# mll-lab-nu/TStar

Hardware: AMD Instinct MI355X
Metric: candidate frames scored/sec (whole node) + sec/video to 8 keyframes, 1h@1fps (higher is better)
Workload: dtype f32 held exactly as 3 bf16 terms per operand: every GEMM and vision-attention operand (activations, weights, Q, K, V, softmax probabilities) = three round-to-nearest bf16 terms carrying all 24 significand bits; the 6 partial products with i + j <= 2 (each exact) on v_mfma_f32_32x32x16_bf16, f32 accu

## Files before the change

### include/tstar_hip.h

```cpp
#ifndef TSTAR_HIP_H
#define TSTAR_HIP_H

#include <stddef.h>
#include <stdint.h>

#ifdef __cplusplus
extern "C" {
#endif

#define TSTAR_OK 0
#define TSTAR_ERR_ARG 1
#define TSTAR_ERR_HIP 2
#define TSTAR_ERR_STATE 3

#define TSTAR_OWL_NPATCH 576
#define TSTAR_OWL_QDIM 512
#define TSTAR_OWL_TEXT_LEN 16
#define TSTAR_OWL_MAX_QUERIES 32
#define TSTAR_OWL_MAX_SETS 64

const char* tstar_last_error(void);
int tstar_abi_version(void);
size_t tstar_owl_vision_blob_floats(void);
size_t tstar_owl_text_blob_floats(void);
// ... 109 lines not shown
int tstar_draw_boxes_np(uint8_t* d_images, int B, int H, int W, const float* d_boxes_xyxy, const float* d_scores, int np,
                        void* stream);

int tstar_gemm_f32(const float* d_A, const float* d_W, float* d_C, const float* d_bias, const float* d_residual,
                   int M, int N, int K, int act, void* stream);
int tstar_gemm_f32_cfg(const float* d_A, const float* d_W, float* d_C, const float* d_bias, const float* d_residual,
                       int M, int N, int K, int act, int tile_cfg, void* stream);
int tstar_gemm_bf16w(const float* d_A, const float* d_W, float* d_C, const float* d_bias, const float* d_residual,
                     int M, int N, int K, int act, int tile_cfg, void* stream);
int tstar_gemm_bf16w2(const float* d_A, const float* d_W, float* d_C, const float* d_bias, const float* d_residual,
                      int M, int N, int K, int act, int tile_cfg, void* stream);
int tstar_gemm_bf16w_pre(const float* d_A, const void* d_Wb, float* d_C, const float* d_bias, const float* d_residual,
                         int M, int N, int K, int act, int a_terms, int tile_cfg, void* stream);
int tstar_gemm_f32x3(const float* d_A, const float* d_W, float* d_C, const float* d_bias, const float* d_residual,
                     int M, int N, int K, int act, int tile_cfg, void* stream);
int tstar_pack_f32x3(const float* d_W, void* d_Wp, int N, int K, void* stream);
int tstar_gemm_f32x3_pre(const float* d_A, const void* d_Wp, float* d_C, const float* d_bias, const float* d_residual,
                         int M, int N, int K, int act, int tile_cfg, void* stream);
int tstar_gemm_plan(int weights_mode, int M, int N, int ldc, int patch_np, int tile_cfg, int has_packed_w2, int* plan4);
int tstar_ingest_plan(int op, int nv12, int H, int W, int n, int ow, int oh, int out_aligned4, int video_aligned4, int generic,
                      int nv12_lds, int grid_px, int* plan6);
int tstar_layernorm_f32(const float* d_x, float* d_y, const float* d_w, const float* d_b, int rows, int D, void* stream);
int tstar_attention_f32(const float* d_qkv, float* d_out, int B, int T, int heads, int mode,
                        const uint8_t* d_key_mask, void* stream);

int tstar_attention_split(const float* d_qkv, float* d_out, int B, int T, int heads, void* stream);
int tstar_attention_x3(const float* d_qkv, float* d_out, int B, int T, int heads, void* stream);

int tstar_prof_enable(int on);
int tstar_prof_read(int category, long long* launches, double* total_ms, double* total_flops);
// ... 9 lines not shown
```

### tstar_amd/_lib.py

```python
from __future__ import annotations

import ctypes as C
import os

_HERE = os.path.dirname(os.path.abspath(__file__))
LIB_PATH = os.path.join(_HERE, "libtstar_hip.so")


class TStarHipError(RuntimeError):
    pass


_vp, _i, _sz = C.c_void_p, C.c_int, C.c_size_t
_fp = C.POINTER(C.c_float)
SIGNATURES = {
    "tstar_last_error": (C.c_char_p, []),
    "tstar_abi_version": (_i, []),
    "tstar_owl_vision_blob_floats": (_sz, []),
    "tstar_owl_text_blob_floats": (_sz, []),
    "tstar_owl_create": (_i, [C.POINTER(_vp), _vp, _sz, _vp, _sz, _vp, _i, _i]),
    "tstar_owl_create_ex": (_i, [C.POINTER(_vp), _i, _i, _vp, _sz, _vp, _sz, _vp, _i, _i]),
    "tstar_owl_vision_blob_floats_ex": (_sz, [_i, _i]),
    "tstar_owl_create_in": (_i, [C.POINTER(_vp), _i, _i, _i, _vp, _sz, _vp, _sz, _vp, _i, _i]),
    "tstar_owl_vision_blob_floats_in": (_sz, [_i, _i, _i]),
# ... 40 lines not shown
    "tstar_searcher_read_state": (_i, [_vp, _vp, _vp]),
    "tstar_searcher_read": (_i, [_vp, _i, _vp, _vp]),
    "tstar_comm_available": (_i, []),
    "tstar_comm_unique_id": (_i, [_vp]),
    "tstar_comm_create": (_i, [C.POINTER(_vp), _vp, _i, _i]),
    "tstar_comm_destroy": (_i, [_vp]),
    "tstar_allgather_i32": (_i, [_vp, _vp, _vp, _i, _vp]),
    "tstar_topk_seconds": (_i, [_vp, _i, _i, _i, _i, _vp, _vp]),
    "tstar_ssim_pairwise": (_i, [_vp, _i, _vp, _i, _i, _i, _vp, _vp, _vp]),
    "tstar_gemm_f32": (_i, [_vp, _vp, _vp, _vp, _vp, _i, _i, _i, _i, _vp]),
    "tstar_gemm_f32_cfg": (_i, [_vp, _vp, _vp, _vp, _vp, _i, _i, _i, _i, _i, _vp]),
    "tstar_gemm_bf16w": (_i, [_vp, _vp, _vp, _vp, _vp, _i, _i, _i, _i, _i, _vp]),
    "tstar_gemm_bf16w2": (_i, [_vp, _vp, _vp, _vp, _vp, _i, _i, _i, _i, _i, _vp]),
    "tstar_gemm_bf16w_pre": (_i, [_vp, _vp, _vp, _vp, _vp, _i, _i, _i, _i, _i, _i, _vp]),
    "tstar_gemm_f32x3": (_i, [_vp, _vp, _vp, _vp, _vp, _i, _i, _i, _i, _i, _vp]),
    "tstar_pack_f32x3": (_i, [_vp, _vp, _i, _i, _vp]),
    "tstar_gemm_f32x3_pre": (_i, [_vp, _vp, _vp, _vp, _vp, _i, _i, _i, _i, _i, _vp]),
    "tstar_gemm_plan": (_i, [_i, _i, _i, _i, _i, _i, _i, C.POINTER(_i)]),
    "tstar_ingest_plan": (_i, [_i] * 12 + [C.POINTER(_i)]),
    "tstar_layernorm_f32": (_i, [_vp, _vp, _vp, _vp, _i, _i, _vp]),
    "tstar_draw_boxes": (_i, [_vp, _i, _i, _i, _vp, _vp, _vp]),
    "tstar_draw_boxes_np": (_i, [_vp, _i, _i, _i, _vp, _vp, _i, _vp]),
    "tstar_attention_split": (_i, [_vp, _vp, _i, _i, _i, _vp]),
    "tstar_attention_x3": (_i, [_vp, _vp, _i, _i, _i, _vp]),
    "tstar_attention_f32": (_i, [_vp, _vp, _i, _i, _i, _i, _vp, _vp]),
    "tstar_prof_enable": (_i, [_i]),
    "tstar_prof_read": (_i, [_i, _vp, _vp, _vp]),
    "tstar_prof_read_bytes": (_i, [_i, _vp]),
    "tstar_prof_read_totals": (_i, [_i, _vp, _vp]),
    "tstar_prof_mark": (_i, [_i, _vp]),
# ... 41 lines not shown
```

### tstar_amd/csrc/capi.hip

```cpp
#include "../../include/tstar_hip.h"
#include "common.h"
#include "heads.h"
#include "ingest.h"
#include "jpeg_host.h"
#include "kernels.h"
#include "owl_weights.h"
#include <math.h>
#include <map>
#include <mutex>
#include <set>
#include <string.h>
#include <unordered_map>
#include <vector>

namespace tstar {
static thread_local std::string g_err;
void set_error(const std::string& msg) { g_err = msg; }

int ensure_dyn_lds(const void* kernel, int bytes) {
    static std::mutex mu;
    static std::set<std::pair<const void*, int>> done;
    int dev = 0;
    if (hipGetDevice(&dev) != hipSuccess) { set_error("ensure_dyn_lds: hipGetDevice failed"); return 2; }
    std::lock_guard<std::mutex> lk(mu);
// ... 48 lines not shown
struct tstar_owl {
    float* d_vision = nullptr;
    float* d_text = nullptr;
    VisionW vw{};
    TextW tw{};
    bool has_text = false, has_vision = false;
    OwlGeom geom{};
    float* d_lut = nullptr;
    int max_batch = 0;
    int chunk_cap = 0;
    size_t mpad = 0;
    struct Lane {
        float *x = nullptr, *xn = nullptr, *qkv = nullptr, *att = nullptr, *hid = nullptr;
        uint8_t* tmp_u8 = nullptr; size_t tmp_u8_bytes = 0;
        int* d_image_set = nullptr; int image_set_cap = 0;
        int cap = 0;
    } lane[TSTAR_OWL_LANES];
    int Q[TSTAR_OWL_MAX_SETS] = {0};
    float *q_raw = nullptr, *qn = nullptr;
    double* qweight = nullptr;
    uint8_t* qmask = nullptr;
    int* d_setQ = nullptr;
    int *d_ids = nullptr, *d_eos = nullptr;
    uint8_t* d_kmask = nullptr;
    int seq_cap = TSTAR_OWL_MAX_QUERIES;
    std::map<std::pair<int, int>, ResampleTable> tabs;
    int weights_mode = TSTAR_WEIGHTS_F32;
    std::unordered_map<const float*, __bf16*> wb;
    std::unordered_map<const float*, void*> wp;
    std::unordered_map<const float*, void*> wq;
// ... 73 lines not shown

static GemmArgs mk_gemm(const tstar_owl* h, const float* A, const float* W, float* C, const float* bias, const float* res,
                        int M, int N, int K, int lda, int ldc, int act) {
    GemmArgs g{};
    g.A = A; g.W = W; g.Wb = h ? h->bf16_of(W) : nullptr; g.Wp = h ? h->packed_of(W) : nullptr; g.Wq = h ? h->w2_of(W) : nullptr; g.C = C; g.bias = bias; g.res = res; g.pos = nullptr;
    g.M = M; g.N = N; g.K = K; g.lda = lda; g.ldc = ldc; g.act = act; g.patch_np = 0; g.tile_cfg = TILE_AUTO; g.m_split = 0;
    g.a_terms = h && h->weights_mode == TSTAR_WEIGHTS_BF16 ? 2 : 0;
    return g;
}

static bool x3_attention_f32() {
    static const bool v = getenv("TSTAR_X3_ATTN_F32") != nullptr;
    return v;
}

static int run_encoder(tstar_owl* h, tstar_owl::Lane& L, const LayerW* layers, int nlayers, int B, int T, int D, int FF, int heads,
                       int mode, const uint8_t* key_mask, hipStream_t s) {
    const int M = B * T;
    for (int l = 0; l < nlayers; ++l) {
        const LayerW& w = layers[l];
        RC(layernorm_f32(L.x, L.xn, w.ln1_w, w.ln1_b, M, D, s));
        RC(gemm_f32(mk_gemm(h, L.xn, w.qkv_w, L.qkv, w.qkv_b, nullptr, M, 3 * D, D, D, 3 * D, ACT_NONE), s));
        if (mode == 0 && (h->weights_mode == TSTAR_WEIGHTS_BF16 || h->weights_mode == TSTAR_WEIGHTS_BF16_EXACT)) RC(attention_split(L.qkv, L.att, B, T, heads, s));
        else if (mode == 0 && h->weights_mode == TSTAR_WEIGHTS_F32X3 && !x3_attention_f32()) RC(attention_x3(L.qkv, L.att, B, T, heads, s));
        else RC(attention_f32(L.qkv, L.att, B, T, heads, mode, key_mask, s));
        RC(gemm_f32(mk_gemm(h, L.att, w.out_w, L.x, w.out_b, L.x, M, D, D, D, D, ACT_NONE), s));
        RC(layernorm_f32(L.x, L.xn, w.ln2_w, w.ln2_b, M, D, s));
        RC(gemm_f32(mk_gemm(h, L.xn, w.fc1_w, L.hid, w.fc1_b, nullptr, M, FF, D, D, FF, ACT_QGELU), s));
        RC(gemm_f32(mk_gemm(h, L.hid, w.fc2_w, L.x, w.fc2_b, L.x, M, D, FF, FF, D, ACT_NONE), s));
    }
    return TSTAR_OK;
}

static int preprocess_chunk(tstar_owl* h, tstar_owl::Lane& L, const uint8_t* d_images, int B, int H, int W, uint8_t* out_u8,
                            float* out_patches, hipStream_t s) {
    ResampleTable *th, *tv;
    const OwlGeom& G = h->geom;
    RC(get_table(h, W, G.in_w, &th, s));
    RC(get_table(h, H, G.in_h, &tv, s));
    const size_t need = (size_t)B * H * G.in_w * 3;
    if (need > L.tmp_u8_bytes) {
        TSTAR_HIP_CHECK(hipStreamSynchronize(s));
        if (L.tmp_u8) TSTAR_HIP_CHECK(hipFree(L.tmp_u8));
        L.tmp_u8 = nullptr; L.tmp_u8_bytes = 0;
        TSTAR_HIP_CHECK(hipMalloc(&L.tmp_u8, need));
        L.tmp_u8_bytes = need;
    }
    RC(resample_h_u8(d_images, L.tmp_u8, B, H, W, *th, s));
    RC(resample_v_normalize_patchify(L.tmp_u8, out_patches, out_u8, B, H, G.in_w, *tv, h->d_lut, G.patch, s));
    return TSTAR_OK;
}

static hipError_t alloc_lane(tstar_owl::Lane& L, int cap, const OwlGeom& g) {
    const size_t mp = lane_rows(cap, g);
    hipError_t e = hipSuccess;
    auto alloc = [&](float** p, size_t n) { if (e == hipSuccess) { e = hipMalloc(p, n * sizeof(float)); if (e == hipSuccess) e = hipMemset(*p, 0, n * sizeof(float)); } };
    alloc(&L.x, mp * V_D); alloc(&L.xn, mp * V_D); alloc(&L.qkv, mp * 3 * V_D); alloc(&L.att, mp * V_D); alloc(&L.hid, mp * V_FF);
    if (e == hipSuccess) L.cap = cap;
    return e;
}
static void free_lane(tstar_owl::Lane& L) {
    void* ptrs[] = {L.x, L.xn, L.qkv, L.att, L.hid, L.tmp_u8, L.d_image_set};
    for (void* p : ptrs) if (p) (void)hipFree(p);
    L = tstar_owl::Lane{};
}

extern "C" {

const char* tstar_last_error(void) { return g_err.c_str(); }
int tstar_abi_version(void) { return 3; }
size_t tstar_owl_vision_blob_floats(void) { return vision_floats(OwlGeom{}); }
size_t tstar_owl_text_blob_floats(void) { return text_floats(); }
size_t tstar_owl_vision_blob_floats_ex(int image_size, int patch_size) {
    OwlGeom g;
    if (!owl_geom(image_size, patch_size, &g)) { set_error("tstar_owl_vision_blob_floats_ex: unsupported geometry (image 768, patch 32 or 16)"); return 0; }
    return vision_floats(g);
}
// ... 356 lines not shown
        }
        TSTAR_HIP_CHECK(hipMemcpyAsync(L.d_image_set, h_image_query_set, (size_t)B * sizeof(int), hipMemcpyHostToDevice, s));
    }
    const int ncell = grid_rows * grid_cols;
    const OwlGeom& G = h->geom;
    const int NP = G.np, NTOK = G.ntok, PK = G.patch_k;
    for (int b0 = 0; b0 < B; b0 += L.cap) {
        const int Bc = (B - b0) < L.cap ? (B - b0) : L.cap;
        const int M = Bc * NTOK, MP = Bc * NP;
        RC(preprocess_chunk(h, L, d_images + (size_t)b0 * H * W * 3, Bc, H, W, nullptr, L.hid, s));
        GemmArgs pg = mk_gemm(h, L.hid, h->vw.patch_w, L.x, nullptr, nullptr, MP, V_D, PK, PK, V_D, ACT_NONE);
        pg.pos = h->vw.pos_emb; pg.patch_np = NP;
        RC(gemm_f32(pg, s));
        RC(write_cls_rows(L.x, h->vw.class_emb, h->vw.pos_emb, Bc, NTOK, V_D, s));
        RC(layernorm_f32(L.x, L.x, h->vw.pre_ln_w, h->vw.pre_ln_b, M, V_D, s));
        RC(run_encoder(h, L, h->vw.layers, V_LAYERS, Bc, NTOK, V_D, V_FF, V_HEADS, 0, nullptr, s));
        float* feats = L.xn;
        RC(merge_cls_ln(L.x, feats, h->vw.post_ln_w, h->vw.post_ln_b, h->vw.det_ln_w, h->vw.det_ln_b, Bc, NTOK, V_D, s));
        float* cls = L.att;
        float* bh1 = L.qkv;
        float* bh2 = L.hid;
        RC(gemm_f32(mk_gemm(h, feats, h->vw.cls_w, cls, h->vw.cls_b, nullptr, MP, PROJ, V_D, V_D, PROJ, ACT_NONE), s));
        RC(gemm_f32(mk_gemm(h, feats, h->vw.box0_w, bh1, h->vw.box0_b, nullptr, MP, V_D, V_D, V_D, V_D, ACT_GELU), s));
        RC(gemm_f32(mk_gemm(h, bh1, h->vw.box1_w, bh2, h->vw.box1_b, nullptr, MP, V_D, V_D, V_D, V_D, ACT_GELU), s));
        DetectRowsArgs a{};
        a.feats = feats; a.cls = cls; a.boxh = bh2; a.qn = h->qn; a.qmask = h->qmask;
        a.shift_w = h->vw.shift_w; a.shift_b = h->vw.shift_b; a.scale_w = h->vw.scale_w; a.scale_b = h->vw.scale_b;
        a.box2_w = h->vw.box2_w; a.box2_b = h->vw.box2_b; a.box_bias = h->vw.box_bias;
        a.scores = d_scores + (size_t)b0 * NP;
        a.labels = d_labels + (size_t)b0 * NP;
// ... 125 lines not shown
    void* wp = nullptr;
    TSTAR_HIP_CHECK(hipMalloc(&wp, (size_t)N * K * 6));
    int rc = pack_weights_x3(d_W, wp, N, K, s);
    if (!rc) {
        GemmArgs g = mk_gemm(nullptr, d_A, d_W, d_C, d_bias, d_residual, M, N, K, K, N, act);
        g.Wp = wp;
        g.tile_cfg = tile_cfg;
        rc = gemm_f32(g, s);
    }
    hipError_t e = hipStreamSynchronize(s);
    (void)hipFree(wp);
    if (!rc && e != hipSuccess) { set_error(std::string("tstar_gemm_f32x3: ") + hipGetErrorString(e)); rc = TSTAR_ERR_HIP; }
    return rc;
}

int tstar_pack_f32x3(const float* d_W, void* d_Wp, int N, int K, void* stream) {
    TSTAR_REQUIRE(d_W && d_Wp, "tstar_pack_f32x3: null argument");
    TSTAR_REQUIRE(N > 0 && K > 0, "tstar_pack_f32x3: empty matrix");
    return pack_weights_x3(d_W, d_Wp, N, K, (hipStream_t)stream);
}

int tstar_gemm_f32x3_pre(const float* d_A, const void* d_Wp, float* d_C, const float* d_bias, const float* d_residual, int M, int N,
                         int K, int act, int tile_cfg, void* stream) {
    TSTAR_REQUIRE(d_A && d_Wp && d_C, "tstar_gemm_f32x3_pre: null argument");
    TSTAR_REQUIRE(M > 0 && N > 0 && K > 0 && N % 128 == 0 && K % 32 == 0, "tstar_gemm_f32x3_pre: N must be a multiple of 128, K of 32 (include/tstar_hip.h)");
    GemmArgs g = mk_gemm(nullptr, d_A, reinterpret_cast<const float*>(d_Wp), d_C, d_bias, d_residual, M, N, K, K, N, act);
    g.Wp = d_Wp;
    g.tile_cfg = tile_cfg;
    return gemm_f32(g, (hipStream_t)stream);
}
// ... 54 lines not shown
```

### tstar_amd/csrc/gemm_f32.hip

```cpp
#include "common.h"
#include "kernels.h"
#include "prof.h"
#include <type_traits>
#include <utility>

namespace tstar {

constexpr int BK = 32, LDS_LD = BK + 4;

__device__ __forceinline__ void tile_mn(int tile, int mt, int nt, int gm, int& mi, int& ni) {
    if (gm <= 1) { mi = tile / nt; ni = tile - mi * nt; return; }
    const int per = gm * nt;
    const int sp = tile / per, r = tile - sp * per;
    const int left = mt - sp * gm;
    const int rows = left < gm ? left : gm;
    ni = r / rows;
    mi = sp * gm + (r - ni * rows);
}

__device__ __forceinline__ float epi_act(float v, int act) {
    if (act == ACT_QGELU) return v * __builtin_amdgcn_rcpf(1.0f + __builtin_amdgcn_exp2f(-1.702f * 1.44269504088896340736f * v));
    if (act == ACT_GELU) return 0.5f * v * (1.0f + erff(v * 0.70710678118654752440f));
    return v;
}
// ... 262 lines not shown
    __syncthreads();
    for (int kt = 0; kt < nk; kt += 2) {
        if (kt + 2 < nk) gload(S0{}, kt + 2);
        compute(0);
        if (kt + 1 < nk) lstore(S1{}, 1);
        __syncthreads();
        if (kt + 1 >= nk) break;
        if (kt + 3 < nk) gload(S1{}, kt + 3);
        compute(1);
        if (kt + 2 < nk) lstore(S0{}, 0);
        __syncthreads();
    }
    gemm_epilogue<CF, ACT, HAS_BIAS, HAS_RES, PATCH>(g, acc, m0, n0, wm, wn, l31, h);
}

template <int NA>
__device__ __forceinline__ void split4_rn(const f32x4 v, u32x2 (&out)[NA]) {
#pragma unroll
    for (int p = 0; p < 2; ++p) {
        f32x2 x; x[0] = v[2 * p]; x[1] = v[2 * p + 1];
#pragma unroll
        for (int k = 0; k < NA; ++k) {
            const bf16x2 b = __builtin_convertvector(x, bf16x2);
            const unsigned hb = __builtin_bit_cast(unsigned, b);
            out[k][p] = hb;
            if (k + 1 < NA) {
                x[0] = x[0] - __uint_as_float(hb << 16);
                x[1] = x[1] - __uint_as_float(hb & 0xFFFF0000u);
            }
        }
// ... 2 lines not shown

__device__ __forceinline__ void split2_rn3(float x0, float x1, unsigned (&o)[3]) {
#pragma unroll
    for (int k = 0; k < 3; ++k) {
        f32x2 x; x[0] = x0; x[1] = x1;
        const unsigned hb = __builtin_bit_cast(unsigned, __builtin_convertvector(x, bf16x2));
        o[k] = hb;
        if (k < 2) {
            x0 = x0 - __uint_as_float(hb << 16);
            x1 = x1 - __uint_as_float(hb & 0xFFFF0000u);
        }
    }
}

template <class CF, int ACT, bool HAS_BIAS, bool HAS_RES, bool PATCH>
__device__ __forceinline__ void gemm_tile_x3(const GemmArgs& g, const int m0, const int n0, float* smem_f) {
    constexpr int TM = CF::TM, TN = CF::TN, BM = CF::BM;
    constexpr int A_T = BM * 64, BUF = 3 * A_T;
    constexpr int NA = BM / 32;
    constexpr int PAIR = TN >= 2 ? 2 : 1, GP = TN / PAIR;
    constexpr int WD = TM * TN == 1 ? 4 : 1;
    static_assert(TN % PAIR == 0, "column tiles go in pairs");
    char* smem = reinterpret_cast<char*>(smem_f);
    const int t = threadIdx.x;
    const int lane = t & 63, wave = __builtin_amdgcn_readfirstlane(t >> 6);
    const int wm = wave >> 1, wn = wave & 1;
    const int l31 = lane & 31, h = lane >> 5;
    const int c4 = t & 7, r0 = t >> 3;
    unsigned aoff[NA];
#pragma unroll
    for (int i = 0; i < NA; ++i) {
// ... 162 lines not shown
        step(std::integral_constant<int, 1>{}, std::integral_constant<int, (s0 + 1) % WD>{}, nxt, rd0, nxt, 2 * kt + 1 + WD, 0);
    };
    if constexpr (WD <= 2) {
        for (int kt = 0; kt < nk; ++kt) tile(std::integral_constant<int, 0>{}, kt);
    } else {
        static_assert(WD == 4, "the loop below is unrolled by WD / 2 = 2 K tiles");
        int kt = 0;
        for (; kt + 1 < nk; kt += 2) {
            tile(std::integral_constant<int, 0>{}, kt);
            tile(std::integral_constant<int, 2>{}, kt + 1);
        }
        if (kt < nk) tile(std::integral_constant<int, 0>{}, kt);
    }
    __builtin_amdgcn_s_setprio(0);
    gemm_epilogue<CF, ACT, HAS_BIAS, HAS_RES, PATCH>(g, acc, m0, n0, wm, wn, l31, h);
}

__global__ __launch_bounds__(256) void pack_x3_kernel(const float* __restrict__ W, char* __restrict__ Wp, int N, int K) {
    const size_t gid = (size_t)blockIdx.x * 256 + threadIdx.x;
    const int kc = K / 8;
    if (gid >= (size_t)N * kc) return;
    const int n = (int)(gid / kc), c = (int)(gid % kc);
    const f32x4 v0 = *reinterpret_cast<const f32x4*>(W + (size_t)n * K + c * 8);
    const f32x4 v1 = *reinterpret_cast<const f32x4*>(W + (size_t)n * K + c * 8 + 4);
    u32x2 s0[3], s1[3];
    split4_rn<3>(v0, s0);
    split4_rn<3>(v1, s1);
    const int ks = c >> 1, hh = c & 1, nph = (K / 16) * 3;
#pragma unroll
    for (int ph = 0; ph < 3; ++ph) {
// ... 258 lines not shown
        __syncthreads();
        cur ^= 1;
    }

    gemm_epilogue<CF, ACT, HAS_BIAS, HAS_RES, PATCH>(g, acc, m0, n0, wm, wn, l31, h);
}

template <class CF, int WMODE, int ACT, bool HAS_BIAS, bool HAS_RES, bool PATCH>
__global__ __launch_bounds__(256, CF::MINW) void gemm_f32_kernel(GemmArgs g) {
    extern __shared__ __attribute__((aligned(16))) float smem[];
    const int nt = g.N / CF::BN;
    const int mt = (g.M + CF::BM - 1) / CF::BM;
    const int tile = xcd_remap(blockIdx.x, mt * nt);
    int mi, ni;
    tile_mn(tile, mt, nt, g.group_m, mi, ni);
    if constexpr (WMODE == 4) gemm_tile_x3<CF, ACT, HAS_BIAS, HAS_RES, PATCH>(g, mi * CF::BM, ni * CF::BN, smem);
    else if constexpr (WMODE != 0) gemm_tile_bf16w<CF, WMODE, ACT, HAS_BIAS, HAS_RES, PATCH>(g, mi * CF::BM, ni * CF::BN, smem);
    else gemm_tile<CF, ACT, HAS_BIAS, HAS_RES, PATCH>(g, mi * CF::BM, ni * CF::BN, smem);
}

template <int WMODE, int ACT, bool HAS_BIAS, bool HAS_RES, bool PATCH>
__global__ __launch_bounds__(256, 2) void gemm_f32_hybrid_kernel(GemmArgs g) {
    extern __shared__ __attribute__((aligned(16))) float smem[];
    const int nt = g.N / 128;
    const int n_big = (g.m_split / 128) * nt;
    if ((int)blockIdx.x < n_big) {
        const int tile = xcd_remap(blockIdx.x, n_big);
        int mi, ni;
        tile_mn(tile, g.m_split / 128, nt, g.group_m, mi, ni);
        if constexpr (WMODE == 4) gemm_tile_x3<Cfg128, ACT, HAS_BIAS, HAS_RES, PATCH>(g, mi * 128, ni * 128, smem);
        else if constexpr (WMODE != 0) gemm_tile_bf16w<Cfg128, WMODE, ACT, HAS_BIAS, HAS_RES, PATCH>(g, mi * 128, ni * 128, smem);
        else gemm_tile<Cfg128, ACT, HAS_BIAS, HAS_RES, PATCH>(g, mi * 128, ni * 128, smem);
    } else {
        const int n_small = gridDim.x - n_big;
        const int tile = xcd_remap(blockIdx.x - n_big, n_small);
        int mi, ni;
        tile_mn(tile, n_small / nt, nt, g.group_m, mi, ni);
        if constexpr (WMODE == 4) gemm_tile_x3<Cfg64N, ACT, HAS_BIAS, HAS_RES, PATCH>(g, g.m_split + mi * 64, ni * 128, smem);
        else if constexpr (WMODE != 0) gemm_tile_bf16w<Cfg64N, WMODE, ACT, HAS_BIAS, HAS_RES, PATCH>(g, g.m_split + mi * 64, ni * 128, smem);
        else gemm_tile<Cfg64N, ACT, HAS_BIAS, HAS_RES, PATCH>(g, g.m_split + mi * 64, ni * 128, smem);
    }
}

template <int WMODE, int ACT, bool HAS_BIAS, bool HAS_RES, bool PATCH, bool VW = false>
__global__ __launch_bounds__(256, 2) void gemm_bf16w2_wide_kernel(GemmArgs g) {
    extern __shared__ __attribute__((aligned(16))) float smem[];
    const int ntw = g.N / 256;
    const int n_big = (g.m_split / 128) * ntw;
    if ((int)blockIdx.x < n_big) {
        const int tile = xcd_remap(blockIdx.x, n_big);
        int mi, ni;
        tile_mn(tile, g.m_split / 128, ntw, g.group_m, mi, ni);
        if constexpr (WMODE == 4) gemm_tile_x3<Cfg128W, ACT, HAS_BIAS, HAS_RES, PATCH>(g, mi * 128, ni * 256, smem);
        else if constexpr (VW) gemm_tile_w2v<Cfg128W, ACT, HAS_BIAS, HAS_RES, PATCH>(g, mi * 128, ni * 256, smem);
        else gemm_tile_bf16w<Cfg128W, 3, ACT, HAS_BIAS, HAS_RES, PATCH>(g, mi * 128, ni * 256, smem);
    } else {
        const int nt = g.N / 128;
        const int n_small = gridDim.x - n_big;
        const int tile = xcd_remap(blockIdx.x - n_big, n_small);
        int mi, ni;
        tile_mn(tile, n_small / nt, nt, g.group_m, mi, ni);
        if constexpr (WMODE == 4) gemm_tile_x3<Cfg64N, ACT, HAS_BIAS, HAS_RES, PATCH>(g, g.m_split + mi * 64, ni * 128, smem);
        else gemm_tile_bf16w<Cfg64N, 3, ACT, HAS_BIAS, HAS_RES, PATCH>(g, g.m_split + mi * 64, ni * 128, smem);
    }
}

static constexpr int lds_bytes(int wmode, int bm, int bn) {
    return wmode == GEMM_W_F32X3 ? 2 * 3 * bm * 64 : wmode == GEMM_W_BF16_2T ? 2 * (2 * bm + bn) * 64 : wmode == GEMM_W_BF16_EXACT ? 2 * (3 * bm + bn) * 64 : 2 * (bm + bn) * LDS_LD * 4;
}

static double gemm_algorithmic_bytes(const GemmArgs& g) {
    const double wbytes = g.Wp ? 6.0 : g.Wb ? 2.0 : 4.0;
    return 4.0 * g.M * g.K + wbytes * g.N * g.K + 4.0 * g.M * g.N * (g.res ? 2.0 : 1.0) + (g.bias ? 4.0 * g.N : 0.0) +
           (g.pos ? 4.0 * (g.patch_np + 1) * g.N : 0.0);
}

static int pick_cfg(int M, int N, int* m_split) {
// ... 94 lines not shown
}

template <int ACT, bool HAS_BIAS, bool HAS_RES, bool PATCH>
static int launch_one(const GemmArgs& g, hipStream_t stream) {
    if (g.Wp) return launch_mode<GEMM_W_F32X3, ACT, HAS_BIAS, HAS_RES, PATCH>(g, stream);
    if (g.Wb && g.a_terms == 2) return launch_mode<GEMM_W_BF16_2T, ACT, HAS_BIAS, HAS_RES, PATCH>(g, stream);
    if (g.Wb) return launch_mode<GEMM_W_BF16_EXACT, ACT, HAS_BIAS, HAS_RES, PATCH>(g, stream);
    return launch_mode<GEMM_W_F32, ACT, HAS_BIAS, HAS_RES, PATCH>(g, stream);
}

static int default_group_m() {
    static const int gm = [] { const char* e = getenv("TSTAR_GEMM_GM"); const int v = e ? atoi(e) : 8; return v < 1 ? 1 : (v > 64 ? 64 : v); }();
    return gm;
}

int gemm_f32(const GemmArgs& g0, hipStream_t stream) {
    GemmArgs g = g0;
    if (g.group_m <= 0) g.group_m = default_group_m();
    TSTAR_REQUIRE(g.M > 0 && g.N > 0 && g.K > 0, "gemm_f32: empty problem");
    TSTAR_REQUIRE(g.K % BK == 0, "gemm_f32: K must be a multiple of 32");
    TSTAR_REQUIRE(g.lda % 4 == 0 && g.K % 4 == 0, "gemm_f32: rows must be 16-byte aligned");
    const bool bias = g.bias != nullptr, res = g.res != nullptr, patch = g.pos != nullptr;
    if (patch) {
        TSTAR_REQUIRE(!bias && !res && g.act == ACT_NONE && g.patch_np > 0, "gemm_f32: patch epilogue takes no bias/res/act");
        return launch_one<ACT_NONE, false, false, true>(g, stream);
    }
    if (g.act == ACT_QGELU) {
        TSTAR_REQUIRE(bias && !res, "gemm_f32: quick-gelu epilogue needs bias, no residual");
        return launch_one<ACT_QGELU, true, false, false>(g, stream);
    }
    if (g.act == ACT_GELU) {
        TSTAR_REQUIRE(bias && !res, "gemm_f32: gelu epilogue needs bias, no residual");
        return launch_one<ACT_GELU, true, false, false>(g, stream);
// ... 9 lines not shown
```

### tstar_amd/csrc/kernels.h

```cpp
#pragma once
#include "common.h"

namespace tstar {

enum { ACT_NONE = 0, ACT_QGELU = 1, ACT_GELU = 2 };

struct GemmArgs {
    const float* A;
    const float* W;
    const __bf16* Wb;
    const void* Wp;
    const void* Wq;
    float* C;
    const float* bias;
    const float* res;
    const float* pos;
    int M, N, K, lda, ldc;
    int act;
    int patch_np;
    int tile_cfg;
    int m_split;
    int group_m;
    int a_terms;
};
int gemm_f32(const GemmArgs& g, hipStream_t stream);

enum GemmTileCfg {
    TILE_AUTO = -1,
    TILE_128 = 0,
    TILE_64N = 1,
    TILE_64 = 2,
    TILE_HYBRID = 3,
    TILE_WIDE = 4,
    TILE_NO_WIDE = 5,
    TILE_WIDE_VW = 6,
    TILE_HYBRID_N = 16,
};

enum GemmWeightMode {
    GEMM_W_F32 = 0,
// ... 46 lines not shown
```

### tstar_amd/csrc/rowops.hip

```cpp
#include "common.h"
#include "kernels.h"

namespace tstar {

__device__ __forceinline__ float wave_sum(float v) {
#pragma unroll
    for (int o = 32; o > 0; o >>= 1) v += __shfl_xor(v, o);
    return v;
}

template <int NV>
__device__ __forceinline__ void ln_regs(f32x4 (&x)[NV], const float* __restrict__ w, const float* __restrict__ b,
                                        int lane, float invD) {
    float s = 0.f;
#pragma unroll
    for (int i = 0; i < NV; ++i) s += (x[i][0] + x[i][1]) + (x[i][2] + x[i][3]);
    const float mean = wave_sum(s) * invD;
    float v = 0.f;
#pragma unroll
    for (int i = 0; i < NV; ++i)
#pragma unroll
        for (int e = 0; e < 4; ++e) { float d = x[i][e] - mean; v += d * d; }
    const float rstd = 1.0f / sqrtf(wave_sum(v) * invD + 1e-5f);
#pragma unroll
    for (int i = 0; i < NV; ++i) {
        const f32x4 wv = *reinterpret_cast<const f32x4*>(w + (i * 64 + lane) * 4);
        const f32x4 bv = *reinterpret_cast<const f32x4*>(b + (i * 64 + lane) * 4);
#pragma unroll
        for (int e = 0; e < 4; ++e) x[i][e] = (x[i][e] - mean) * rstd * wv[e] + bv[e];
    }
}

template <int NV>
__global__ __launch_bounds__(256) void layernorm_kernel(const float* __restrict__ x, float* __restrict__ y,
                                                        const float* __restrict__ w, const float* __restrict__ b,
                                                        int rows) {
    const int lane = threadIdx.x & 63;
    const int row = blockIdx.x * 4 + (threadIdx.x >> 6);
    if (row >= rows) return;
    constexpr int D = NV * 256;
    f32x4 v[NV];
#pragma unroll
    for (int i = 0; i < NV; ++i) v[i] = *reinterpret_cast<const f32x4*>(x + (size_t)row * D + (i * 64 + lane) * 4);
    ln_regs<NV>(v, w, b, lane, 1.0f / D);
#pragma unroll
    for (int i = 0; i < NV; ++i) *reinterpret_cast<f32x4*>(y + (size_t)row * D + (i * 64 + lane) * 4) = v[i];
}

int layernorm_f32(const float* x, float* y, const float* w, const float* b, int rows, int D, hipStream_t s) {
    TSTAR_REQUIRE(rows > 0, "layernorm_f32: no rows");
    const int grid = cdiv(rows, 4);
    if (D == 768) hipLaunchKernelGGL(layernorm_kernel<3>, dim3(grid), dim3(256), 0, s, x, y, w, b, rows);
    else if (D == 512) hipLaunchKernelGGL(layernorm_kernel<2>, dim3(grid), dim3(256), 0, s, x, y, w, b, rows);
    else { TSTAR_REQUIRE(false, "layernorm_f32: D must be 512 or 768"); }
    TSTAR_HIP_CHECK(hipGetLastError());
    return TSTAR_OK;
}

__global__ void cls_rows_kernel(float* __restrict__ x, const float* __restrict__ cls, const float* __restrict__ pos,
                                int ntok, int D) {
    const int b = blockIdx.x;
// ... 48 lines not shown
```

Baseline: 11990.

## Fuse LayerNorm into residual GEMM epilogue via last-tile atomic ticket

Adds an optional LayerNorm tail to the f32x3 GEMM. Each output tile bumps a per-row-block atomic counter, and the block that finishes last for that row band computes LayerNorm over the full 768-wide rows and writes them to xn. This applies to the out-projection (ln2) and to fc2 (the next layer's ln1), removing two standalone LayerNorm launches and their extra pass over x per layer. The cost is serialized LN work inside the last-arriving block, plus a counter memset and the added release/acquire fences.

```diff
diff --git a/include/tstar_hip.h b/include/tstar_hip.h
--- a/include/tstar_hip.h
+++ b/include/tstar_hip.h
@@ -147,6 +147,9 @@
                          int M, int N, int K, int act, int a_terms, int tile_cfg, void* stream);
 int tstar_gemm_f32x3(const float* d_A, const float* d_W, float* d_C, const float* d_bias, const float* d_residual,
                      int M, int N, int K, int act, int tile_cfg, void* stream);
+int tstar_gemm_f32x3_ln(const float* d_A, const float* d_W, float* d_C, const float* d_bias, const float* d_residual,
+                        const float* d_ln_w, const float* d_ln_b, float* d_ln_out, int* d_ln_cnt, int M, int N, int K,
+                        int tile_cfg, void* stream);
 int tstar_pack_f32x3(const float* d_W, void* d_Wp, int N, int K, void* stream);
 int tstar_gemm_f32x3_pre(const float* d_A, const void* d_Wp, float* d_C, const float* d_bias, const float* d_residual,
                          int M, int N, int K, int act, int tile_cfg, void* stream);
diff --git a/tstar_amd/_lib.py b/tstar_amd/_lib.py
--- a/tstar_amd/_lib.py
+++ b/tstar_amd/_lib.py
@@ -78,6 +78,7 @@
     "tstar_gemm_bf16w2": (_i, [_vp, _vp, _vp, _vp, _vp, _i, _i, _i, _i, _i, _vp]),
     "tstar_gemm_bf16w_pre": (_i, [_vp, _vp, _vp, _vp, _vp, _i, _i, _i, _i, _i, _i, _vp]),
     "tstar_gemm_f32x3": (_i, [_vp, _vp, _vp, _vp, _vp, _i, _i, _i, _i, _i, _vp]),
+    "tstar_gemm_f32x3_ln": (_i, [_vp, _vp, _vp, _vp, _vp, _vp, _vp, _vp, _vp, _i, _i, _i, _i, _vp]),
     "tstar_pack_f32x3": (_i, [_vp, _vp, _i, _i, _vp]),
     "tstar_gemm_f32x3_pre": (_i, [_vp, _vp, _vp, _vp, _vp, _i, _i, _i, _i, _i, _vp]),
     "tstar_gemm_plan": (_i, [_i, _i, _i, _i, _i, _i, _i, C.POINTER(_i)]),
diff --git a/tstar_amd/csrc/capi.hip b/tstar_amd/csrc/capi.hip
--- a/tstar_amd/csrc/capi.hip
+++ b/tstar_amd/csrc/capi.hip
@@ -86,6 +86,7 @@
         float *x = nullptr, *xn = nullptr, *qkv = nullptr, *att = nullptr, *hid = nullptr;
         uint8_t* tmp_u8 = nullptr; size_t tmp_u8_bytes = 0;
         int* d_image_set = nullptr; int image_set_cap = 0;
+        int* ln_cnt = nullptr;
         int cap = 0;
     } lane[TSTAR_OWL_LANES];
     int Q[TSTAR_OWL_MAX_SETS] = {0};
@@ -189,20 +190,37 @@
     return v;
 }
 
+static bool ln_fusion_on() {
+    static const bool v = getenv("TSTAR_LN_FUSE_OFF") == nullptr;
+    return v;
+}
+static size_t ln_cnt_bytes(size_t M) { return round_up((size_t)gemm_ln_counters((int)M) * sizeof(int), 16); }
+
+static bool fuse_ln(GemmArgs& g, const tstar_owl::Lane& L, const float* ln_w, const float* ln_b, int D) {
+    if (!ln_fusion_on() || !L.ln_cnt || !gemm_ln_fusable(g)) return false;
+    g.ln_w = ln_w; g.ln_b = ln_b; g.ln_out = L.xn; g.ln_ld = D; g.ln_cnt = L.ln_cnt;
+    return true;
+}
+
 static int run_encoder(tstar_owl* h, tstar_owl::Lane& L, const LayerW* layers, int nlayers, int B, int T, int D, int FF, int heads,
                        int mode, const uint8_t* key_mask, hipStream_t s) {
     const int M = B * T;
+    bool xn_ready = false;
     for (int l = 0; l < nlayers; ++l) {
         const LayerW& w = layers[l];
-        RC(layernorm_f32(L.x, L.xn, w.ln1_w, w.ln1_b, M, D, s));
+        if (!xn_ready) RC(layernorm_f32(L.x, L.xn, w.ln1_w, w.ln1_b, M, D, s));
         RC(gemm_f32(mk_gemm(h, L.xn, w.qkv_w, L.qkv, w.qkv_b, nullptr, M, 3 * D, D, D, 3 * D, ACT_NONE), s));
         if (mode == 0 && (h->weights_mode == TSTAR_WEIGHTS_BF16 || h->weights_mode == TSTAR_WEIGHTS_BF16_EXACT)) RC(attention_split(L.qkv, L.att, B, T, heads, s));
         else if (mode == 0 && h->weights_mode == TSTAR_WEIGHTS_F32X3 && !x3_attention_f32()) RC(attention_x3(L.qkv, L.att, B, T, heads, s));
         else RC(attention_f32(L.qkv, L.att, B, T, heads, mode, key_mask, s));
-        RC(gemm_f32(mk_gemm(h, L.att, w.out_w, L.x, w.out_b, L.x, M, D, D, D, D, ACT_NONE), s));
-        RC(layernorm_f32(L.x, L.xn, w.ln2_w, w.ln2_b, M, D, s));
+        GemmArgs og = mk_gemm(h, L.att, w.out_w, L.x, w.out_b, L.x, M, D, D, D, D, ACT_NONE);
+        const bool ln2_fused = fuse_ln(og, L, w.ln2_w, w.ln2_b, D);
+        RC(gemm_f32(og, s));
+        if (!ln2_fused) RC(layernorm_f32(L.x, L.xn, w.ln2_w, w.ln2_b, M, D, s));
         RC(gemm_f32(mk_gemm(h, L.xn, w.fc1_w, L.hid, w.fc1_b, nullptr, M, FF, D, D, FF, ACT_QGELU), s));
-        RC(gemm_f32(mk_gemm(h, L.hid, w.fc2_w, L.x, w.fc2_b, L.x, M, D, FF, FF, D, ACT_NONE), s));
+        GemmArgs fg = mk_gemm(h, L.hid, w.fc2_w, L.x, w.fc2_b, L.x, M, D, FF, FF, D, ACT_NONE);
+        xn_ready = l + 1 < nlayers && fuse_ln(fg, L, layers[l + 1].ln1_w, layers[l + 1].ln1_b, D);
+        RC(gemm_f32(fg, s));
     }
     return TSTAR_OK;
 }
@@ -231,11 +249,12 @@
     hipError_t e = hipSuccess;
     auto alloc = [&](float** p, size_t n) { if (e == hipSuccess) { e = hipMalloc(p, n * sizeof(float)); if (e == hipSuccess) e = hipMemset(*p, 0, n * sizeof(float)); } };
     alloc(&L.x, mp * V_D); alloc(&L.xn, mp * V_D); alloc(&L.qkv, mp * 3 * V_D); alloc(&L.att, mp * V_D); alloc(&L.hid, mp * V_FF);
+    if (e == hipSuccess) { e = hipMalloc(&L.ln_cnt, ln_cnt_bytes(mp)); if (e == hipSuccess) e = hipMemset(L.ln_cnt, 0, ln_cnt_bytes(mp)); }
     if (e == hipSuccess) L.cap = cap;
     return e;
 }
 static void free_lane(tstar_owl::Lane& L) {
-    void* ptrs[] = {L.x, L.xn, L.qkv, L.att, L.hid, L.tmp_u8, L.d_image_set};
+    void* ptrs[] = {L.x, L.xn, L.qkv, L.att, L.hid, L.ln_cnt, L.tmp_u8, L.d_image_set};
     for (void* p : ptrs) if (p) (void)hipFree(p);
     L = tstar_owl::Lane{};
 }
@@ -622,6 +641,7 @@
         RC(gemm_f32(pg, s));
         RC(write_cls_rows(L.x, h->vw.class_emb, h->vw.pos_emb, Bc, NTOK, V_D, s));
         RC(layernorm_f32(L.x, L.x, h->vw.pre_ln_w, h->vw.pre_ln_b, M, V_D, s));
+        if (ln_fusion_on()) TSTAR_HIP_CHECK(hipMemsetAsync(L.ln_cnt, 0, ln_cnt_bytes((size_t)M), s));
         RC(run_encoder(h, L, h->vw.layers, V_LAYERS, Bc, NTOK, V_D, V_FF, V_HEADS, 0, nullptr, s));
         float* feats = L.xn;
         RC(merge_cls_ln(L.x, feats, h->vw.post_ln_w, h->vw.post_ln_b, h->vw.det_ln_w, h->vw.det_ln_b, Bc, NTOK, V_D, s));
@@ -777,6 +797,27 @@
     return rc;
 }
 
+int tstar_gemm_f32x3_ln(const float* d_A, const float* d_W, float* d_C, const float* d_bias, const float* d_residual, const float* d_ln_w,
+                        const float* d_ln_b, float* d_ln_out, int* d_ln_cnt, int M, int N, int K, int tile_cfg, void* stream) {
+    TSTAR_REQUIRE(d_A && d_W && d_C && d_bias && d_residual && d_ln_w && d_ln_b && d_ln_out && d_ln_cnt, "tstar_gemm_f32x3_ln: null argument");
+    TSTAR_REQUIRE(M > 0 && N == 768 && K > 0 && K % 32 == 0, "tstar_gemm_f32x3_ln: N must be 768, K a multiple of 32 (include/tstar_hip.h)");
+    hipStream_t s = (hipStream_t)stream;
+    void* wp = nullptr;
+    TSTAR_HIP_CHECK(hipMalloc(&wp, (size_t)N * K * 6));
+    int rc = pack_weights_x3(d_W, wp, N, K, s);
+    if (!rc) {
+        GemmArgs g = mk_gemm(nullptr, d_A, d_W, d_C, d_bias, d_residual, M, N, K, K, N, ACT_NONE);
+        g.Wp = wp;
+        g.tile_cfg = tile_cfg;
+        g.ln_w = d_ln_w; g.ln_b = d_ln_b; g.ln_out = d_ln_out; g.ln_ld = N; g.ln_cnt = d_ln_cnt;
+        rc = gemm_f32(g, s);
+    }
+    hipError_t e = hipStreamSynchronize(s);
+    (void)hipFree(wp);
+    if (!rc && e != hipSuccess) { set_error(std::string("tstar_gemm_f32x3_ln: ") + hipGetErrorString(e)); rc = TSTAR_ERR_HIP; }
+    return rc;
+}
+
 int tstar_pack_f32x3(const float* d_W, void* d_Wp, int N, int K, void* stream) {
     TSTAR_REQUIRE(d_W && d_Wp, "tstar_pack_f32x3: null argument");
     TSTAR_REQUIRE(N > 0 && K > 0, "tstar_pack_f32x3: empty matrix");
diff --git a/tstar_amd/csrc/gemm_f32.hip b/tstar_amd/csrc/gemm_f32.hip
--- a/tstar_amd/csrc/gemm_f32.hip
+++ b/tstar_amd/csrc/gemm_f32.hip
@@ -1,5 +1,6 @@
 #include "common.h"
 #include "kernels.h"
+#include "ln_rows.h"
 #include "prof.h"
 #include <type_traits>
 #include <utility>
@@ -300,6 +301,32 @@
     gemm_epilogue<CF, ACT, HAS_BIAS, HAS_RES, PATCH>(g, acc, m0, n0, wm, wn, l31, h);
 }
 
+template <int BM>
+__device__ __forceinline__ void gemm_ln_tail(const GemmArgs& g, const int m0, const int cnt_idx, const int tickets, float* smem_f,
+                                             const int wave, const int lane) {
+    typedef __attribute__((address_space(1))) int gint;
+    asm volatile("s_waitcnt vmcnt(0)" ::: "memory");
+    __syncthreads();
+    __attribute__((address_space(3))) int* flag = (__attribute__((address_space(3))) int*)smem_f;
+    if (wave == 0 && lane == 0) {
+        gint* cnt = (gint*)(g.ln_cnt + cnt_idx);
+        __builtin_amdgcn_fence(__ATOMIC_RELEASE, "agent");
+        asm volatile("s_waitcnt vmcnt(0)" ::: "memory");
+        const int ticket = __hip_atomic_fetch_add(cnt, 1, __ATOMIC_RELAXED, __HIP_MEMORY_SCOPE_AGENT);
+        const int last = ticket == tickets - 1;
+        if (last) {
+            __hip_atomic_store(cnt, 0, __ATOMIC_RELAXED, __HIP_MEMORY_SCOPE_AGENT);
+            __builtin_amdgcn_fence(__ATOMIC_ACQUIRE, "agent");
+            asm volatile("s_waitcnt vmcnt(0)" ::: "memory");
+        }
+        *flag = last;
+    }
+    __syncthreads();
+    if (*flag == 0) return;
+    const int end = m0 + BM < g.M ? m0 + BM : g.M;
+    ln_rows<3, BM / 16>(g.C, g.ldc, g.ln_out, g.ln_ld, g.ln_w, g.ln_b, m0 + wave, 4, end, lane);
+}
+
 template <int NA>
 __device__ __forceinline__ void split4_rn(const f32x4 v, u32x2 (&out)[NA]) {
 #pragma unroll
@@ -332,7 +359,7 @@
 }
 
 template <class CF, int ACT, bool HAS_BIAS, bool HAS_RES, bool PATCH>
-__device__ __forceinline__ void gemm_tile_x3(const GemmArgs& g, const int m0, const int n0, float* smem_f) {
+__device__ __forceinline__ void gemm_tile_x3(const GemmArgs& g, const int m0, const int n0, float* smem_f, const int ln_idx = 0, const int ln_tickets = 0) {
     constexpr int TM = CF::TM, TN = CF::TN, BM = CF::BM;
     constexpr int A_T = BM * 64, BUF = 3 * A_T;
     constexpr int NA = BM / 32;
@@ -525,6 +552,7 @@
     }
     __builtin_amdgcn_s_setprio(0);
     gemm_epilogue<CF, ACT, HAS_BIAS, HAS_RES, PATCH>(g, acc, m0, n0, wm, wn, l31, h);
+    if constexpr (HAS_RES) if (g.ln_out) gemm_ln_tail<BM>(g, m0, ln_idx, ln_tickets, smem_f, wave, l31 + 32 * h);
 }
 
 __global__ __launch_bounds__(256) void pack_x3_kernel(const float* __restrict__ W, char* __restrict__ Wp, int N, int K) {
@@ -813,7 +841,7 @@
     const int tile = xcd_remap(blockIdx.x, mt * nt);
     int mi, ni;
     tile_mn(tile, mt, nt, g.group_m, mi, ni);
-    if constexpr (WMODE == 4) gemm_tile_x3<CF, ACT, HAS_BIAS, HAS_RES, PATCH>(g, mi * CF::BM, ni * CF::BN, smem);
+    if constexpr (WMODE == 4) gemm_tile_x3<CF, ACT, HAS_BIAS, HAS_RES, PATCH>(g, mi * CF::BM, ni * CF::BN, smem, mi, nt);
     else if constexpr (WMODE != 0) gemm_tile_bf16w<CF, WMODE, ACT, HAS_BIAS, HAS_RES, PATCH>(g, mi * CF::BM, ni * CF::BN, smem);
     else gemm_tile<CF, ACT, HAS_BIAS, HAS_RES, PATCH>(g, mi * CF::BM, ni * CF::BN, smem);
 }
@@ -827,7 +855,7 @@
         const int tile = xcd_remap(blockIdx.x, n_big);
         int mi, ni;
         tile_mn(tile, g.m_split / 128, nt, g.group_m, mi, ni);
-        if constexpr (WMODE == 4) gemm_tile_x3<Cfg128, ACT, HAS_BIAS, HAS_RES, PATCH>(g, mi * 128, ni * 128, smem);
+        if constexpr (WMODE == 4) gemm_tile_x3<Cfg128, ACT, HAS_BIAS, HAS_RES, PATCH>(g, mi * 128, ni * 128, smem, mi, nt);
         else if constexpr (WMODE != 0) gemm_tile_bf16w<Cfg128, WMODE, ACT, HAS_BIAS, HAS_RES, PATCH>(g, mi * 128, ni * 128, smem);
         else gemm_tile<Cfg128, ACT, HAS_BIAS, HAS_RES, PATCH>(g, mi * 128, ni * 128, smem);
     } else {
@@ -835,7 +863,7 @@
         const int tile = xcd_remap(blockIdx.x - n_big, n_small);
         int mi, ni;
         tile_mn(tile, n_small / nt, nt, g.group_m, mi, ni);
-        if constexpr (WMODE == 4) gemm_tile_x3<Cfg64N, ACT, HAS_BIAS, HAS_RES, PATCH>(g, g.m_split + mi * 64, ni * 128, smem);
+        if constexpr (WMODE == 4) gemm_tile_x3<Cfg64N, ACT, HAS_BIAS, HAS_RES, PATCH>(g, g.m_split + mi * 64, ni * 128, smem, g.m_split / 128 + mi, nt);
         else if constexpr (WMODE != 0) gemm_tile_bf16w<Cfg64N, WMODE, ACT, HAS_BIAS, HAS_RES, PATCH>(g, g.m_split + mi * 64, ni * 128, smem);
         else gemm_tile<Cfg64N, ACT, HAS_BIAS, HAS_RES, PATCH>(g, g.m_split + mi * 64, ni * 128, smem);
     }
@@ -850,7 +878,7 @@
         const int tile = xcd_remap(blockIdx.x, n_big);
         int mi, ni;
         tile_mn(tile, g.m_split / 128, ntw, g.group_m, mi, ni);
-        if constexpr (WMODE == 4) gemm_tile_x3<Cfg128W, ACT, HAS_BIAS, HAS_RES, PATCH>(g, mi * 128, ni * 256, smem);
+        if constexpr (WMODE == 4) gemm_tile_x3<Cfg128W, ACT, HAS_BIAS, HAS_RES, PATCH>(g, mi * 128, ni * 256, smem, mi, ntw);
         else if constexpr (VW) gemm_tile_w2v<Cfg128W, ACT, HAS_BIAS, HAS_RES, PATCH>(g, mi * 128, ni * 256, smem);
         else gemm_tile_bf16w<Cfg128W, 3, ACT, HAS_BIAS, HAS_RES, PATCH>(g, mi * 128, ni * 256, smem);
     } else {
@@ -859,7 +887,7 @@
         const int tile = xcd_remap(blockIdx.x - n_big, n_small);
         int mi, ni;
         tile_mn(tile, n_small / nt, nt, g.group_m, mi, ni);
-        if constexpr (WMODE == 4) gemm_tile_x3<Cfg64N, ACT, HAS_BIAS, HAS_RES, PATCH>(g, g.m_split + mi * 64, ni * 128, smem);
+        if constexpr (WMODE == 4) gemm_tile_x3<Cfg64N, ACT, HAS_BIAS, HAS_RES, PATCH>(g, g.m_split + mi * 64, ni * 128, smem, g.m_split / 128 + mi, nt);
         else gemm_tile_bf16w<Cfg64N, 3, ACT, HAS_BIAS, HAS_RES, PATCH>(g, g.m_split + mi * 64, ni * 128, smem);
     }
 }
@@ -984,9 +1012,19 @@
     return gm;
 }
 
+bool gemm_ln_fusable(const GemmArgs& g) {
+    return g.Wp != nullptr && g.res != nullptr && g.bias != nullptr && g.pos == nullptr && g.act == ACT_NONE && g.N == 768;
+}
+
 int gemm_f32(const GemmArgs& g0, hipStream_t stream) {
     GemmArgs g = g0;
     if (g.group_m <= 0) g.group_m = default_group_m();
+    if (g.ln_out || g.ln_w || g.ln_b || g.ln_cnt) {
+        TSTAR_REQUIRE(g.ln_out && g.ln_w && g.ln_b && g.ln_cnt, "gemm_f32: the fused LayerNorm needs ln_w, ln_b, ln_out and ln_cnt");
+        TSTAR_REQUIRE(gemm_ln_fusable(g), "gemm_f32: the fused LayerNorm needs the f32x3 mode, bias + residual, no activation and N = 768");
+        TSTAR_REQUIRE(g.ln_ld >= g.N && g.ln_ld % 4 == 0 && g.ldc % 4 == 0, "gemm_f32: fused LayerNorm rows must be 16-byte aligned");
+        TSTAR_REQUIRE(g.ln_out != g.C && g.ln_out != g.res && g.ln_out != g.A, "gemm_f32: ln_out must not alias an operand of the launch");
+    }
     TSTAR_REQUIRE(g.M > 0 && g.N > 0 && g.K > 0, "gemm_f32: empty problem");
     TSTAR_REQUIRE(g.K % BK == 0, "gemm_f32: K must be a multiple of 32");
     TSTAR_REQUIRE(g.lda % 4 == 0 && g.K % 4 == 0, "gemm_f32: rows must be 16-byte aligned");
diff --git a/tstar_amd/csrc/kernels.h b/tstar_amd/csrc/kernels.h
--- a/tstar_amd/csrc/kernels.h
+++ b/tstar_amd/csrc/kernels.h
@@ -22,8 +22,16 @@
     int m_split;
     int group_m;
     int a_terms;
+    const float* ln_w;
+    const float* ln_b;
+    float* ln_out;
+    int* ln_cnt;
+    int ln_ld;
 };
 int gemm_f32(const GemmArgs& g, hipStream_t stream);
+
+bool gemm_ln_fusable(const GemmArgs& g);
+static inline int gemm_ln_counters(int M) { return cdiv(M, 64); }
 
 enum GemmTileCfg {
     TILE_AUTO = -1,
diff --git a/tstar_amd/csrc/ln_rows.h b/tstar_amd/csrc/ln_rows.h
--- /dev/null
+++ b/tstar_amd/csrc/ln_rows.h
@@ -0,0 +1,60 @@
+#pragma once
+#include "common.h"
+
+namespace tstar {
+
+__device__ __forceinline__ float wave_sum(float v) {
+#pragma unroll
+    for (int o = 32; o > 0; o >>= 1) v += __shfl_xor(v, o);
+    return v;
+}
+
+template <int NV>
+__device__ __forceinline__ void ln_regs(f32x4 (&x)[NV], const float* __restrict__ w, const float* __restrict__ b,
+                                        int lane, float invD) {
+    float s = 0.f;
+#pragma unroll
+    for (int i = 0; i < NV; ++i) s += (x[i][0] + x[i][1]) + (x[i][2] + x[i][3]);
+    const float mean = wave_sum(s) * invD;
+    float v = 0.f;
+#pragma unroll
+    for (int i = 0; i < NV; ++i)
+#pragma unroll
+        for (int e = 0; e < 4; ++e) { float d = x[i][e] - mean; v += d * d; }
+    const float rstd = 1.0f / sqrtf(wave_sum(v) * invD + 1e-5f);
+#pragma unroll
+    for (int i = 0; i < NV; ++i) {
+        const f32x4 wv = *reinterpret_cast<const f32x4*>(w + (i * 64 + lane) * 4);
+        const f32x4 bv = *reinterpret_cast<const f32x4*>(b + (i * 64 + lane) * 4);
+#pragma unroll
+        for (int e = 0; e < 4; ++e) x[i][e] = (x[i][e] - mean) * rstd * wv[e] + bv[e];
+    }
+}
+
+template <int NV, int U>
+__device__ __forceinline__ void ln_rows(const float* x, int ldx, float* y, int ldy, const float* __restrict__ w,
+                                        const float* __restrict__ b, int first, int step, int end, int lane) {
+    constexpr int D = NV * 256;
+    for (int r0 = first; r0 < end; r0 += U * step) {
+        f32x4 v[U][NV];
+#pragma unroll
+        for (int u = 0; u < U; ++u) {
+            const int r = r0 + u * step;
+            const float* xr = x + (size_t)(r < end ? r : first) * ldx;
+#pragma unroll
+            for (int i = 0; i < NV; ++i) v[u][i] = *reinterpret_cast<const f32x4*>(xr + (i * 64 + lane) * 4);
+        }
+#pragma unroll
+        for (int u = 0; u < U; ++u) {
+            ln_regs<NV>(v[u], w, b, lane, 1.0f / D);
+            const int r = r0 + u * step;
+            if (r < end) {
+                float* yr = y + (size_t)r * ldy;
+#pragma unroll
+                for (int i = 0; i < NV; ++i) *reinterpret_cast<f32x4*>(yr + (i * 64 + lane) * 4) = v[u][i];
+            }
+        }
+    }
+}
+
+}
diff --git a/tstar_amd/csrc/rowops.hip b/tstar_amd/csrc/rowops.hip
--- a/tstar_amd/csrc/rowops.hip
+++ b/tstar_amd/csrc/rowops.hip
@@ -1,35 +1,8 @@
 #include "common.h"
 #include "kernels.h"
+#include "ln_rows.h"
 
 namespace tstar {
-
-__device__ __forceinline__ float wave_sum(float v) {
-#pragma unroll
-    for (int o = 32; o > 0; o >>= 1) v += __shfl_xor(v, o);
-    return v;
-}
-
-template <int NV>
-__device__ __forceinline__ void ln_regs(f32x4 (&x)[NV], const float* __restrict__ w, const float* __restrict__ b,
-                                        int lane, float invD) {
-    float s = 0.f;
-#pragma unroll
-    for (int i = 0; i < NV; ++i) s += (x[i][0] + x[i][1]) + (x[i][2] + x[i][3]);
-    const float mean = wave_sum(s) * invD;
-    float v = 0.f;
-#pragma unroll
-    for (int i = 0; i < NV; ++i)
-#pragma unroll
-        for (int e = 0; e < 4; ++e) { float d = x[i][e] - mean; v += d * d; }
-    const float rstd = 1.0f / sqrtf(wave_sum(v) * invD + 1e-5f);
-#pragma unroll
-    for (int i = 0; i < NV; ++i) {
-        const f32x4 wv = *reinterpret_cast<const f32x4*>(w + (i * 64 + lane) * 4);
-        const f32x4 bv = *reinterpret_cast<const f32x4*>(b + (i * 64 + lane) * 4);
-#pragma unroll
-        for (int e = 0; e < 4; ++e) x[i][e] = (x[i][e] - mean) * rstd * wv[e] + bv[e];
-    }
-}
 
 template <int NV>
 __global__ __launch_bounds__(256) void layernorm_kernel(const float* __restrict__ x, float* __restrict__ y,
@@ -39,12 +12,7 @@
     const int row = blockIdx.x * 4 + (threadIdx.x >> 6);
     if (row >= rows) return;
     constexpr int D = NV * 256;
-    f32x4 v[NV];
-#pragma unroll
-    for (int i = 0; i < NV; ++i) v[i] = *reinterpret_cast<const f32x4*>(x + (size_t)row * D + (i * 64 + lane) * 4);
-    ln_regs<NV>(v, w, b, lane, 1.0f / D);
-#pragma unroll
-    for (int i = 0; i < NV; ++i) *reinterpret_cast<f32x4*>(y + (size_t)row * D + (i * 64 + lane) * 4) = v[i];
+    ln_rows<NV, 1>(x, D, y, D, w, b, row, 1, row + 1, lane);
 }
 
 int layernorm_f32(const float* x, float* y, const float* w, const float* b, int rows, int D, hipStream_t s) {
```

After: 11780. -1.8%, worse.
